# lyclyc52/SANeRF-HQ

Hardware: AMD Instinct MI355X
Metric: rays/s full render (800x800, hashgrid L=16 + 2x64 MLP) (higher is better)
Workload: dtype f32 arithmetic / f16 tables

## Files before the change

### include/sanerf_hip.h

```cpp
#ifndef SANERF_HIP_H
#define SANERF_HIP_H

#include <stddef.h>
#include <stdint.h>

#ifdef __cplusplus
extern "C" {
#endif

#define SN_MAX_LEVELS 32
#define SN_MAX_LAYERS 8
#define SN_MAX_STAGES 4
#define SN_ABI_VERSION 12

typedef void *sn_stream_t;

typedef enum {
    SN_OK = 0,
    SN_ERR_INVALID = -1,
    SN_ERR_UNSUPPORTED = -2,
    SN_ERR_HIP = -3,
    SN_ERR_WORKSPACE = -4,
    SN_ERR_WINDOW = -5
} sn_status;
// ... 249 lines not shown
    float       *f_feat;
    uint32_t     head_stride;
    void        *workspace;
    size_t       workspace_bytes;
} sn_render_io;

size_t sn_rm_render_workspace_bytes(const sn_render_cfg *cfg, uint32_t N, uint32_t tile_w);
int sn_rm_render_rays(const sn_render_cfg *cfg, const sn_render_io *io, sn_stream_t stream);
typedef struct sn_launch_info {
    char     final_kernel[64];
    uint32_t workgroups, lds_bytes, dense_levels, gathers_per_wave_sample, launches;
} sn_launch_info;
int sn_rm_last_launch_info(sn_launch_info *info);
int sn_rm_render_route_info(const sn_render_cfg *cfg, const sn_render_io *io, sn_launch_info *out);

int sn_rm_grid_composite(const float *xyzs, const float *weights, uint32_t N, uint32_t T, float bound,
                         const sn_grid_desc *grid, uint32_t tile_w, float *out, sn_stream_t stream);

size_t sn_mlp_wide_workspace_bytes(const sn_mlp_desc *mlp);
int sn_mlp_wide_overflow(int32_t *flag);
int sn_mlp_wide_forward(const sn_mlp_desc *mlp, const float *ln_weight, const float *ln_bias, float ln_eps,
                        const float *x, uint32_t N, float *out, void *workspace, size_t workspace_bytes,
                        sn_stream_t stream);

size_t sn_rm_mask_head_workspace_bytes(const sn_mlp_desc *mlp);
int sn_rm_mask_head(const float *xyzs, const float *extra, const float *weights, uint32_t N, uint32_t T, uint32_t E,
                    float bound, const sn_grid_desc *grid, const sn_mlp_desc *mlp, float *out,
                    void *workspace, size_t workspace_bytes, sn_stream_t stream);

int sn_mlp_wide_forward_train(const sn_mlp_desc *mlp, const float *x, uint32_t N, float *const *hidden, float *out, sn_stream_t stream);
// ... 58 lines not shown
```

### sanerf-hq_amd/_lib.py

```python
from __future__ import annotations

import ctypes as C
import os
import subprocess
from typing import Optional

import torch

_PKG = os.path.dirname(os.path.abspath(__file__))
LIB_PATH = os.environ.get("SN_LIB") or os.path.join(_PKG, "libsanerf_hip.so")
CSRC = os.path.join(_PKG, "csrc")

MAX_LEVELS, MAX_LAYERS, MAX_STAGES = 32, 8, 4
SN_F32, SN_F16 = 0, 1
LAYOUT_LBC, LAYOUT_BLC = 0, 1


class GridDesc(C.Structure):
    _fields_ = [("embeddings", C.c_void_p), ("table_dtype", C.c_int32), ("offsets", C.c_int32 * (MAX_LEVELS + 1)),
                ("D", C.c_uint32), ("C", C.c_uint32), ("L", C.c_uint32), ("S", C.c_float), ("H", C.c_uint32),
                ("gridtype", C.c_uint32), ("align_corners", C.c_uint32), ("interp", C.c_uint32)]


class MlpDesc(C.Structure):
# ... 29 lines not shown
                ("pred", C.c_uint64 * MASK_MAX_CLASSES), ("truth", C.c_uint64 * MASK_MAX_CLASSES)]


class SsimRecord(C.Structure):
    _fields_ = [("ssim_sum", C.c_double), ("last", C.c_double), ("images", C.c_uint64)]


class RenderTuning(C.Structure):
    _fields_ = [("mlp_mode", C.c_int32), ("per_sample_form", C.c_int32), ("densify", C.c_int32), ("linear_tile_order", C.c_int32),
                ("prop_sp_max_rays", C.c_int32), ("final_sp_max_rays", C.c_int32), ("feat_levels", C.c_int32), ("band_streams", C.c_int32), ("exact_early_out", C.c_int32), ("wave_tile", C.c_int32), ("prop_sp_lanes", C.c_int32), ("feat_patch", C.c_int32), ("prop_pair", C.c_int32), ("experiment", C.c_int32)]


class LaunchInfo(C.Structure):
    _fields_ = [("final_kernel", C.c_char * 64), ("workgroups", C.c_uint32), ("lds_bytes", C.c_uint32), ("dense_levels", C.c_uint32),
                ("gathers_per_wave_sample", C.c_uint32), ("launches", C.c_uint32)]


class RenderCfg(C.Structure):
    _fields_ = [("num_stages", C.c_uint32), ("num_steps", C.c_uint32 * MAX_STAGES),
                ("prop_grid", GridDesc * MAX_STAGES), ("prop_mlp", MlpDesc * MAX_STAGES),
                ("grid", GridDesc), ("grid_mlp", MlpDesc), ("view_mlp", MlpDesc),
                ("sh_degree", C.c_uint32), ("aabb", C.c_float * 6), ("min_near", C.c_float), ("bound", C.c_float),
                ("contract", C.c_int32), ("last_sample_opaque", C.c_int32), ("bg_color", C.c_float),
                ("feat_grid", GridDesc), ("with_feat", C.c_int32), ("early_stop_eps", C.c_float), ("mlp_exact_fp32", C.c_int32),
                ("compact_live", C.c_int32), ("tuning", RenderTuning)]


class RenderIO(C.Structure):
    _fields_ = [("rays_o", C.c_void_p), ("rays_d", C.c_void_p), ("cam_near_far", C.c_void_p),
                ("N", C.c_uint32), ("tile_w", C.c_uint32),
# ... 74 lines not shown
    "sn_rm_mask_nll": (_int, [_vp, _vp, _u32, _u32, _f32, _vp, _vp, _vp]),
    "sn_rm_ray_pair_select": (_int, [_vp, _vp, _u32, _u32, _u32, _vp, _vp]),
    "sn_rm_ray_pair_rgb_loss": (_int, [_vp, _vp, _int, _vp, _u32, _u32, _u32, _u32, _f32, _f32, _f32, _int, _f32, _vp, _vp, _vp, _vp, _vp]),
    "sn_rm_mask_error": (_int, [_vp, _int, _vp, _u32, _u32, _f32, _f32, _vp, _vp]),
    "sn_rm_error_map_update": (_int, [_vp, _int, _vp, _vp, _u32, _vp, _u32, _u32, _f32, _f32, _u32, _u32, _vp, _vp, _vp, _vp]),
    "sn_rm_mask_output": (_int, [_vp, _u32, _u32, _vp, _u32, _vp, _u32, _int, _int, _f32, _vp, _vp, _vp, _vp, _vp, _vp, _vp]),
    "sn_rm_mask_eval_accumulate": (_int, [_vp, _vp, _u32, _u32, _u32, _f32, _vp, _vp, _vp]),
    "sn_rm_image_sqerr_accumulate": (_int, [_vp, _u32, _vp, _u32, _u32, _vp, _vp, _vp]),
    "sn_rm_image_ssim_accumulate": (_int, [_vp, _u32, _vp, _u32, _u32, _u32, _f32, _vp, _vp, _vp]),
    "sn_rm_feature_distill_workspace_bytes": (C.c_size_t, [_u32, _u32, _u32, _u32, _u32]),
    "sn_rm_feature_distill_loss": (_int, [_vp, _u32, _u32, _u32, _u32, _vp, _u32, _u32, _f32, _vp, _vp, _vp, _vp, _vp, C.c_size_t, _vp]),
    "sn_rm_feature_map": (_int, [_vp, _u32, _u32, _u32, _u32, _u32, _u32, _vp, _vp]),
    "sn_rm_debug_occupancy": (_int, [_vp, _vp, _int]),
    "sn_rm_last_launch_info": (_int, [_vp]),
    "sn_rm_render_route_info": (_int, [C.POINTER(RenderCfg), C.POINTER(RenderIO), _vp]),
    "sn_debug_eval": (_int, [_int, _vp, _vp, _u32, _vp, _vp]),
}

EXPORTED_SYMBOLS = tuple(_SIGNATURES)

_lib = None


def build(force: bool = False) -> str:
    srcs = [os.path.join(CSRC, f) for f in os.listdir(CSRC) if f.endswith((".hip", ".h", ".inc"))]
    srcs.append(os.path.join(os.path.dirname(_PKG), "include", "sanerf_hip.h"))
    stale = force or not os.path.exists(LIB_PATH) or os.path.getmtime(LIB_PATH) < max(os.path.getmtime(s) for s in srcs)
    if stale:
        subprocess.check_call(["make", "-C", CSRC, "-j4"] + (["-B"] if force else []))
    return LIB_PATH
# ... 54 lines not shown
```

### sanerf-hq_amd/csrc/render.hip

```cpp
#include "sn_common.h"
#include "sh_basis.inc"

#include <float.h>
#include <stdlib.h>
#include <string.h>
#include <cstdio>
#include <map>
#include <mutex>
#include <type_traits>
#include <vector>

namespace sn {

typedef float floatx16 __attribute__((ext_vector_type(16)));

struct RayCommon {
    const float *rays_o, *rays_d, *cnf;
    uint32_t N;
    uint32_t W;
    uint32_t rows;
    uint32_t Npad;
    float aabb[6];
    float min_near, bound;
    int contract, last_opaque;
// ... 2958 lines not shown
struct WorkspacePlan {
    BandPlan bands;
    size_t pair_main = 0, pair_prop[SN_MAX_STAGES] = {};
    size_t pair_floats = 0, slot_floats = 0;
    size_t head_floats() const { return (size_t)PACK_FLOATS + pair_floats; }
    size_t bytes() const { return ((size_t)bands.slots * slot_floats + head_floats()) * sizeof(float); }
};
struct RenderRoute {
    GridLevels gl_prop[SN_MAX_STAGES], gl_main, gl_feat;
    bool is_main = false, is_any = false;
    AnyShape any;
    int mlp_mode = MLP_F16X3, mlp_np = 3;
    bool use_cmp = false;
    int Kmain = -1;
    int Kv_main = 0;
    float stop_cum = 0.0f;
    WorkspacePlan ws;
    FinalRoute fin;
    FeatRoute feat;
    uint32_t chunks = 0;
    ChunkRoute full, last;
};

static WorkspacePlan plan_workspace(const sn_render_cfg *cfg, uint32_t N, uint32_t W) {
    WorkspacePlan w;
    w.bands = band_plan(cfg, N, W);
    const uint32_t nc = w.bands.chunk < N ? w.bands.chunk : N;
    w.slot_floats = stage_scratch_floats(cfg, blocks_for(nc, W, tile_log2w(cfg)) * 256u);
    w.pair_floats = w.pair_main = pair_floats_of(&cfg->grid, (uint64_t)N * cfg->num_steps[cfg->num_stages - 1], cfg->tuning.densify);
    for (uint32_t k = 0; k + 1 < cfg->num_stages; ++k) w.pair_floats += w.pair_prop[k] = pair_floats_of(&cfg->prop_grid[k]);
// ... 2 lines not shown

static int check_io_pointers(const sn_render_cfg *cfg, const sn_render_io *io) {
    SN_REQUIRE(io->rays_o && io->rays_d, "render_rays: rays must be device pointers");
    if (io->skip_final) SN_REQUIRE(cfg->num_stages >= 2 && (cfg->num_stages > SN_MAX_STAGES  || io->bins[cfg->num_stages - 1]) && !cfg->with_feat,
                                   "render_rays: skip_final needs >= 2 stages, io->bins[last] for the resampled bins, and no feature stage");
    else SN_REQUIRE(io->image && io->depth && io->weights_sum, "render_rays: outputs must be device pointers");
    return SN_OK;
}

static void plan_final(const sn_render_cfg *cfg, const sn_render_io *io, RenderRoute *r) {
    const uint32_t S = cfg->num_stages;
    const bool f16 = cfg->grid.table_dtype == SN_F16;
    const int dp = dense_prefix(r->gl_main);
    const uint64_t main_samples = (uint64_t)io->N * cfg->num_steps[S - 1];
    r->Kv_main = r->is_any ? 0 : dp;
    const bool have_pairs = !r->is_any && dp > 0 && r->ws.pair_main != 0;
    r->Kmain = have_pairs && final_lv_fits(r->gl_main, dp, 2u * (f16 ? 2u : 4u)) ? dp : -1;
    if (cfg->compact_live && r->mlp_mode == MLP_F16X3 && !cfg->with_feat && !io->xyzs_last && !io->geo_feat_last && !io->skip_final &&
        io->bins0_ray_stride == 0) {
        bool any_dbg = false;
        for (uint32_t k = 1; k < S; ++k) any_dbg = any_dbg || io->u_ray_stride[k] != 0;
        for (uint32_t k = 0; k < S; ++k) any_dbg = any_dbg || io->bins[k] || io->weights[k] || io->sigmas[k] || io->inds[k];
        r->use_cmp = !any_dbg && dp == 5 && r->Kmain == 5;
    }
    if (io->skip_final) return;
    const bool dbg_last = io->bins[S - 1] || io->weights[S - 1] || io->sigmas[S - 1] || io->xyzs_last || io->geo_feat_last;
    const bool per_sample_out = dbg_last || cfg->with_feat;
    r->stop_cum = (cfg->early_stop_eps > 0.0f && cfg->early_stop_eps < 1.0f && !per_sample_out) ? -logf(cfg->early_stop_eps) : 0.0f;
    auto lv_gathers = [&](int kd) -> uint32_t { return (uint32_t)kd * (f16 ? 2u : 4u) + (uint32_t)(16 - kd) * 8u; };
    FinalRoute &f = r->fin;
    f.f16 = f16;
    f.aux = cfg->with_feat || r->stop_cum > 0.0f;
    f.eo = cfg->tuning.exact_early_out == 2;
    const int xp = experiment_of(cfg);
    const bool f16x3 = r->mlp_mode == MLP_F16X3;
    if (r->is_any) {
        f.family = FinalRoute::ANY; f.name = "k_final_stage_any";
        f.lds = (size_t)(2u * r->any.rows + (r->any.dg[r->any.ng] - 1u)) * 256u * sizeof(float);
        f.dense = 0; f.gathers = cfg->grid.L * 8u;
    } else if (r->use_cmp) {
        f.family = FinalRoute::CMP; f.name = "k_final_stage_cmp"; f.K = 5; f.lds = LDS_F16X3; f.dense = 5; f.gathers = lv_gathers(5);
    } else if (f16x3 && r->Kmain == 5 && !f.aux && !per_sample_out && xp == SN_EXP_ROLE_SPLIT) {
        f.family = FinalRoute::RS; f.name = "k_final_stage_rs"; f.K = 5; f.dense = 5; f.gathers = lv_gathers(5);
    } else if (f16x3 && r->Kmain == 5 && !dbg_last && lt_enabled(cfg)) {
        const bool l0 = f16 && (uint64_t)r->gl_main.res[0] * r->gl_main.res[0] * r->gl_main.res[0] <= (uint64_t)L0_MAX_ROWS && xp == SN_EXP_LDS_LEVEL0;
        if (!f.aux && !cfg->compact_live) r->Kv_main = densify_levels(r->gl_main, 5, main_samples, f16, cfg->tuning.densify);
        const bool dens = r->Kv_main == 7 && !l0 && final_lv_fits(r->gl_main, 7, 2u * (f16 ? 2u : 4u));
        f.family = l0 ? FinalRoute::LT_L0 : FinalRoute::LT;
        f.K = dens ? 7 : 5;
        f.name = l0 ? "k_final_stage<lt,K=5,lds-level0>" : dens ? "k_final_stage<lt,K=7>" : f.aux ? "k_final_stage<lt,K=5,aux>" : "k_final_stage<lt,K=5>";
        f.dense = f.K; f.gathers = lv_gathers(f.K) - (l0 ? 2u : 0u);
        if (f16 && !f.eo && r->mlp_np == 1 && !f.aux && !l0) f.np = 1;
        f.lds = l0 ? LDS_F16X3_L0 : (xp == SN_EXP_FINAL_ONE_WG && !dens && f.np == 3) ? (size_t)(84 * 1024) : LDS_F16X3;
    } else if (f16x3) {
        f.family = FinalRoute::PER_SAMPLE; f.K = r->Kmain == 5 ? 5 : -1; f.lds = LDS_F16X3;
        f.name = r->Kmain == 5 ? "k_final_stage<per-sample,K=5>" : "k_final_stage<per-sample,generic>";
        f.dense = r->Kmain; f.gathers = r->Kmain == 5 ? lv_gathers(5) : (uint32_t)dp * 4u + (16u - (uint32_t)dp) * 8u;
    } else if (r->mlp_mode == MLP_F32) {
        f.family = FinalRoute::MFMA32; f.name = "k_final_stage<mfma32>"; f.aux = true; f.lds = LDS_MFMA32; f.dense = -1; f.gathers = 16u * 8u;
    } else {
        f.family = FinalRoute::VALU; f.name = "k_final_stage<valu>"; f.aux = true; f.lds = LDS_VALU; f.dense = -1; f.gathers = 16u * 8u;
// ... 38 lines not shown
        sp.lds = final_sp_lds_floats(1u << spl_log2) * sizeof(float);
        sp.dense = r.Kmain; sp.gathers = r.Kmain == 5 ? (uint32_t)5 * (f.f16 ? 2u : 4u) + 11u * 8u : 16u * 8u;
        f = sp;
    }
    return c;
}

static void plan_chunks(const sn_render_cfg *cfg, const sn_render_io *io, RenderRoute *r) {
    const uint32_t chunk = r->ws.bands.chunk;
    r->chunks = div_up(io->N, chunk);
    r->full = plan_chunk(cfg, io, *r, io->N < chunk ? io->N : chunk);
    const uint32_t n_last = io->N - (r->chunks - 1u) * chunk;
    r->last = n_last == r->full.n ? r->full : plan_chunk(cfg, io, *r, n_last);
}

static int plan_render(const sn_render_cfg *cfg, const sn_render_io *io, RenderRoute *r) {
    SN_REQUIRE(io->out_stride == 0u || io->out_stride >= 5u, "render_rays: out_stride %u must be 0 (dense outputs) or at least 5 floats (rgb | depth | weights_sum per row)", io->out_stride);
    SN_REQUIRE(io->head_stride == 0u || (io->f_image && io->head_stride >= 31u + 4u && !io->skip_final),
               "render_rays: head_stride %u needs f_image and room for f_image | rgb | depth (>= 35 floats per row)", io->head_stride);
    SN_REQUIRE(cfg->tuning.wave_tile >= 0 && cfg->tuning.wave_tile <= 5, "render_rays: tuning.wave_tile %d outside 0..5", cfg->tuning.wave_tile);
    SN_REQUIRE(!(experiment_of(cfg) == SN_EXP_ROLE_SPLIT && cfg->tuning.wave_tile != 0 && cfg->tuning.wave_tile != 3), "render_rays: the role-split experiment is built for 8x8 wave tiles (tuning.wave_tile 0 or 3)");
    const uint32_t S = cfg->num_stages;
    SN_REQUIRE(S >= 1 && S <= SN_MAX_STAGES, "render_rays: num_stages=%u outside 1..%d", S, SN_MAX_STAGES);
    for (uint32_t k = 0; k < S; ++k) SN_REQUIRE(cfg->num_steps[k] >= 1, "render_rays: num_steps[%u] must be >= 1", k);
    SN_REQUIRE(cfg->sh_degree == 4, "render_rays: fused path is built for SH degree 4 (network.py:97), got %u", cfg->sh_degree);
    if (io->tile_w) SN_REQUIRE(io->N % io->tile_w == 0, "render_rays: N=%u is not a multiple of tile_w=%u", io->N, io->tile_w);
    SN_REQUIRE(io->bins0_ray_stride == 0 || (io->bins0_table && io->bins0_ray_stride >= cfg->num_steps[0] + 1u),
               "render_rays: bins0_ray_stride=%u needs bins0_table and at least num_steps[0]+1=%u values per ray", io->bins0_ray_stride, cfg->num_steps[0] + 1u);
    for (uint32_t k = 1; k < S; ++k)
        SN_REQUIRE(io->u_ray_stride[k] == 0 || (io->u_table[k] && io->u_ray_stride[k] >= cfg->num_steps[k] + 1u),
                   "render_rays: u_ray_stride[%u]=%u needs u_table[%u] and at least num_steps[%u]+1=%u values per ray", k, io->u_ray_stride[k], k, k, cfg->num_steps[k] + 1u);
// ... 174 lines not shown
        if (lg == 4u) return k_feat_stage<TT, C, 4, true>;
        if (lg == 2u) return k_feat_stage<TT, C, 2, true>;
        return k_feat_stage<TT, C, 1, true>;
    }
    if (lg == 4u) return k_feat_stage<TT, C, 4>;
    if (lg == 2u) return k_feat_stage<TT, C, 2>;
    return k_feat_stage<TT, C, 1>;
}
static FeatKern feat_kernel(const FeatRoute &ft, bool patch) {
    switch (ft.C) {
        case 8: return ft.f16 ? feat_kernel_of<__half, 8>(ft.lg, patch) : feat_kernel_of<float, 8>(ft.lg, patch);
        case 4: return ft.f16 ? feat_kernel_of<__half, 4>(ft.lg, patch) : feat_kernel_of<float, 4>(ft.lg, patch);
        default: return ft.f16 ? feat_kernel_of<__half, 2>(ft.lg, patch) : feat_kernel_of<float, 2>(ft.lg, patch);
    }
}
}

extern "C" {

size_t sn_rm_render_workspace_bytes(const sn_render_cfg *cfg, uint32_t N, uint32_t tile_w) {
    if (!cfg || N == 0 || cfg->num_stages < 1 || cfg->num_stages > SN_MAX_STAGES) return (size_t)PACK_FLOATS * sizeof(float);
    return plan_workspace(cfg, N, tile_w).bytes();
}

int sn_rm_render_route_info(const sn_render_cfg *cfg, const sn_render_io *io, sn_launch_info *out) {
    SN_REQUIRE(cfg && io && out, "render_route_info: cfg/io/out is NULL");
    *out = sn_launch_info{};
    if (io->N == 0) return SN_OK;
    int rc = check_io_pointers(cfg, io);
    if (rc) return rc;
    RenderRoute route;
    rc = plan_render(cfg, io, &route);
    if (rc) return rc;
    if (io->skip_final) return SN_OK;
    note_final(route.last.fin, out);
    out->launches = route.chunks;
    return SN_OK;
}

int sn_rm_render_rays(const sn_render_cfg *cfg, const sn_render_io *io, sn_stream_t stream) {
    SN_REQUIRE(cfg && io, "render_rays: cfg/io is NULL");
    if (io->N == 0) return SN_OK;
    g_launch = sn_launch_info{};
    int rc = check_io_pointers(cfg, io);
    if (rc) return rc;
    RenderRoute route;
    rc = plan_render(cfg, io, &route);
    if (rc) return rc;
    SN_REQUIRE(io->workspace != nullptr, "render_rays: workspace is NULL");
    SN_REQUIRE(table_aligned(io->workspace), "render_rays: workspace must be 16-byte aligned");
    if (io->workspace_bytes / sizeof(float) < route.ws.bytes() / sizeof(float)) {
        set_error("render_rays: workspace too small (%zu bytes, need %zu)", io->workspace_bytes, route.ws.bytes());
        return SN_ERR_WORKSPACE;
    }
    const uint32_t S = cfg->num_stages, W = io->tile_w;
    const hipStream_t st_main = (hipStream_t)stream;
    const GridLevels &gl_main = route.gl_main;
    float *pack = reinterpret_cast<float *>(io->workspace);
    float *pair_mem = pack + PACK_FLOATS;
    float *scratch = pair_mem + route.ws.pair_floats;

    if (route.mlp_mode != MLP_VALU && !route.is_any) {
        ProfScope ps(st_main, PK_PACK);
        if (route.mlp_mode == MLP_F16X3)
            rc = launch(k_pack_grid_mlp_f16, dim3(PACK16_VECS * 64 / 256), dim3(256), 0, st_main, cfg->grid_mlp.weight[0], cfg->grid_mlp.weight[1],
                        cfg->grid_mlp.weight[2], reinterpret_cast<uint4 *>(pack));
        else
            rc = launch(k_pack_grid_mlp, dim3(PACK_FLOATS / 256), dim3(256), 0, st_main, cfg->grid_mlp.weight[0], cfg->grid_mlp.weight[1], cfg->grid_mlp.weight[2], pack);
        if (rc) return rc;
        SN_LAUNCH_CHECK("k_pack_grid_mlp");
    }
    PairTab pairs, prop_pairs[SN_MAX_STAGES];
    {
        float *cursor = pair_mem;
        auto pack_pairs = [&](const sn_grid_desc *d, const GridLevels &gl, PairTab &pt, int Kp, size_t fl) -> int {
            pt.base = nullptr;
            for (int l = 0; l < 8; ++l) pt.off[l] = 0;
            if (fl == 0 || Kp <= 0) return SN_OK;
            pair_layout(gl, Kp, pt.off);
            pt.base = cursor;
            cursor += fl;
            uint32_t max_rows = 0;
            for (int l = 0; l < Kp; ++l) { const uint32_t r3 = gl.res[l] * gl.res[l] * gl.res[l]; if (r3 > max_rows) max_rows = r3; }
            const dim3 gp(div_up(max_rows, 256), (uint32_t)Kp);
            const int rcl = d->table_dtype == SN_F16 ? launch(k_pack_pairs<__half>, gp, dim3(256), 0, st_main, (const __half *)d->embeddings, gl, pt, (uint32_t)Kp)
                                                     : launch(k_pack_pairs<float>, gp, dim3(256), 0, st_main, (const float *)d->embeddings, gl, pt, (uint32_t)Kp);
            if (rcl) return rcl;
            SN_LAUNCH_CHECK("k_pack_pairs");
            return SN_OK;
        };
        ProfScope ps(st_main, PK_PACK);
        rc = pack_pairs(&cfg->grid, gl_main, pairs, route.Kv_main, route.ws.pair_main);
        if (rc) return rc;
        for (uint32_t k = 0; k + 1 < S; ++k) {
            rc = pack_pairs(&cfg->prop_grid[k], route.gl_prop[k], prop_pairs[k], dense_prefix(route.gl_prop[k]), route.ws.pair_prop[k]);
            if (rc) return rc;
        }
    }

    BandFork fork(st_main, route.ws.bands.slots == 2u);
    if (route.ws.bands.slots == 2u && !fork.side) {
        route.ws.bands.slots = 1u;
        plan_chunks(cfg, io, &route);
    }
    const uint32_t chunk = route.ws.bands.chunk;
    for (uint32_t ci = 0; ci < route.chunks; ++ci) {
        const uint32_t first = ci * chunk;
        const ChunkRoute &cr = ci + 1u < route.chunks ? route.full : route.last;
        const uint32_t n = cr.n, Npad = cr.Npad;
        const uint32_t slot = fork.side ? (ci & 1u) : 0u;
        const hipStream_t st = slot ? fork.side : st_main;
        RayCommon rays;
// ... 90 lines not shown
                ft.level0 = 0;
                rc = launch(feat_kernel(feat, true), dim3(cr.nblk, feat.patch_levels / feat.lg), dim3(256), 0, st, ft);
                if (rc) return rc;
            }
            if (feat.patch_levels < gf.L) {
                ft.level0 = feat.patch_levels;
                rc = launch(feat_kernel(feat, false), dim3(cr.nblk, (gf.L - feat.patch_levels) / feat.lg), dim3(256), 0, st, ft);
                if (rc) return rc;
            }
            SN_LAUNCH_CHECK("k_feat_stage");
        }
    }
    return SN_OK;
}

}
```

### sanerf-hq_amd/raymarching/raymarching.py

```python
from __future__ import annotations

import ctypes as C
import os
import warnings
from typing import Dict, List, Optional, Sequence

import numpy as np
import torch
from torch.autograd import Function

from .. import _lib


class Tuning:
    FIELDS = ("mlp_mode", "per_sample_form", "densify", "linear_tile_order", "prop_sp_max_rays", "final_sp_max_rays", "feat_levels", "band_streams", "exact_early_out", "wave_tile", "prop_sp_lanes", "feat_patch", "prop_pair", "experiment")

    def __init__(self, **kw):
        for f in self.FIELDS:
            setattr(self, f, 0)
        for k, v in kw.items():
            if k not in self.FIELDS:
                raise TypeError(f"Tuning: unknown field {k!r} (fields: {', '.join(self.FIELDS)})")
            setattr(self, k, int(v))

# ... 890 lines not shown
        if feat_encoder is not None:
            _fill_grid(cfg.feat_grid, feat_encoder, table_of(feat_encoder))
            cfg.with_feat = 1
            self.feat_dim = feat_encoder.output_dim
        cfg.early_stop_eps = float(early_stop_eps)
        cfg.compact_live = int(bool(compact_live))
        self.cfg = cfg
        self._range_model = model
        self._range_versions = None
        self.activation_bound = 0.0
        self.check_range()
        self.num_steps = [int(t) for t in num_steps]
        self.geo = int(getattr(model, "geom_feat_dim", list(model.grid_mlp.net)[-1].weight.shape[0] - 1))
        self.ncol = self.geo + model.view_encoder.output_dim
        self._ws: Optional[torch.Tensor] = None

    @torch.no_grad()
    def check_range(self) -> None:
        m = self._range_model
        tensors = [m.grid.embeddings] + [lin.weight for lin in m.grid_mlp.net]
        versions = tuple((t.data_ptr(), t._version) for t in tensors)
        if versions == self._range_versions:
            return
        self._range_versions = versions
        layers = list(m.grid_mlp.net)
        stats = [m.grid.embeddings.detach().abs().max().float()]
        stats += [lin.weight.detach().float().abs().sum(dim=1).max() for lin in layers[:-1]]
        stats += [lin.weight.detach().abs().max().float() for lin in layers]
        vals = torch.stack(stats).tolist()
        bound = worst = vals[0]
        for row_l1 in vals[1:len(layers)]:
            bound = row_l1 * bound
            worst = max(worst, bound)
        wmax = max(vals[len(layers):]) if layers else 0.0
        if any(v != v for v in vals):
            worst = float("nan")
        self.activation_bound = max(worst, wmax)
        exact = not (self.activation_bound < FP16_SPLIT_LIMIT)
        if exact and not self.cfg.mlp_exact_fp32:
            warnings.warn(f"fused render: activations of the 32-64-64-16 MLP are only bounded by {self.activation_bound:.3g} "
                          f"(>= {FP16_SPLIT_LIMIT:.0f}): using the exact fp32 matrix-core path instead of split-fp16")
        self.cfg.mlp_exact_fp32 = int(exact)

    def invalidate_range(self) -> None:
        self._range_versions = None

    @torch.no_grad()
    def refresh_tables(self) -> None:
        for src, copy in self.copies:
            copy.copy_(src.detach())

    def workspace(self, N: int, tile_w: int, device) -> torch.Tensor:
        (self.tuning or tuning).write(self.cfg.tuning)
        need = int(_lib.lib().sn_rm_render_workspace_bytes(C.byref(self.cfg), N, tile_w))
        if self._ws is None or self._ws.numel() < need or self._ws.device != torch.device(device):
            self._ws = torch.empty(need, dtype=torch.uint8, device=device)
        return self._ws


def _fill_io(plan: RenderPlan, io, N: int, tile_w: int, want, u_tables, bins0_table, skip_final: bool, packed, head_input: bool, tuning, buf, table):
    io.N, io.tile_w = N, int(tile_w)
    if bins0_table is not None:
        b0, io.bins0_table = table(bins0_table)
        if b0.dim() == 2:
            if b0.shape != (N, plan.num_steps[0] + 1):
# ... 41 lines not shown
    if head_input and plan.cfg.with_feat and not skip_final:
        io.f_feat = buf("head_input", (N, plan.feat_dim + plan.ncol + 4))
        io.f_image, io.head_stride = io.f_feat + 4 * plan.feat_dim, plan.feat_dim + plan.ncol + 4
    else:
        if "f_image" in want:
            io.f_image = buf("f_image", (N, plan.ncol))
        if plan.cfg.with_feat and not skip_final:
            io.f_feat = buf("f_feat", (N, plan.feat_dim))
    eff = tuning or plan.tuning or globals()["tuning"]
    eff.write(plan.cfg.tuning)
    return eff


def route_info(plan: RenderPlan, N: int, tile_w: int = 0, want: Sequence[str] = (), u_tables: Optional[Dict[int, torch.Tensor]] = None,
               bins0_table: Optional[torch.Tensor] = None, skip_final: bool = False, tuning: Optional["Tuning"] = None,
               packed: Optional[torch.Tensor] = None, head_input: bool = False) -> dict:
    io = _lib.RenderIO()
    stand_in = 64
    io.rays_o = io.rays_d = stand_in
    _fill_io(plan, io, int(N), tile_w, want, u_tables, bins0_table, skip_final, packed, head_input, tuning,
             lambda name, shape, dtype=torch.float32: stand_in, lambda t: (t, stand_in))
    info = _lib.LaunchInfo()
    _lib.check(_lib.lib().sn_rm_render_route_info(C.byref(plan.cfg), C.byref(io), C.byref(info)), "route_info")
    return dict(final_kernel=info.final_kernel.decode(), workgroups=int(info.workgroups), lds_bytes=int(info.lds_bytes),
                dense_levels=int(info.dense_levels), gathers_per_wave_sample=int(info.gathers_per_wave_sample), launches=int(info.launches))


def render_rays(plan: RenderPlan, rays_o, rays_d, cam_near_far=None, bg_color: float = 1.0, tile_w: int = 0,
                want: Sequence[str] = (), u_tables: Optional[Dict[int, torch.Tensor]] = None,
                bins0_table: Optional[torch.Tensor] = None, out: Optional[Dict[str, torch.Tensor]] = None,
                skip_final: bool = False, tuning: Optional["Tuning"] = None, packed: Optional[torch.Tensor] = None,
                head_input: bool = False):
    rays_o, rays_d = _flat3(rays_o), _flat3(rays_d)
    N = rays_o.shape[0]
    device = rays_o.device
    io = _lib.RenderIO()
    res: Dict[str, torch.Tensor] = {} if out is None else out
    keep: List[torch.Tensor] = []

    def buf(name, shape, dtype=torch.float32):
        t = res.get(name)
        if t is None or tuple(t.shape) != tuple(shape) or t.dtype != dtype or t.device != device or not t.is_contiguous():
            t = torch.empty(shape, device=device, dtype=dtype)
            res[name] = t
        return _lib.dev(t, name, dtype)

    def table(t):
# ... 14 lines not shown
                and packed.is_contiguous() and packed.device == device):
            raise RuntimeError(f"render_rays: packed must be a contiguous fp32 [{N}, >=5] tensor on {device}, got {tuple(packed.shape)} {packed.dtype}")
        res["image"], res["depth"], res["weights_sum"] = packed[:, :3], packed[:, 3], packed[:, 4]
    eff = _fill_io(plan, io, N, tile_w, want, u_tables, bins0_table, skip_final, packed, head_input, tuning, buf, table)
    S = plan.cfg.num_stages
    if io.head_stride:
        hb = res["head_input"]
        res["f_feat"], res["f_image"] = hb[:, :plan.feat_dim], hb[:, plan.feat_dim:plan.feat_dim + plan.ncol]
    need = int(_lib.lib().sn_rm_render_workspace_bytes(C.byref(plan.cfg), N, int(tile_w)))
    ws = plan.workspace(N, int(tile_w), device)
    if ws.numel() < need:
        plan._ws = ws = torch.empty(need, dtype=torch.uint8, device=device)
    eff.write(plan.cfg.tuning)
    io.workspace, io.workspace_bytes = ws.data_ptr(), ws.numel()
    plan.cfg.bg_color = float(bg_color)
    _lib.check(_lib.lib().sn_rm_render_rays(C.byref(plan.cfg), C.byref(io), _lib.stream()), "render_rays")
    if "weights_last" in set(want) and not skip_final:
        res["weights_last"] = res[f"weights{S - 1}"]
    return res
```

Before: 102.0 million.

## Cache packed MLP weights and pair tables across render calls

Adds a prepared-state API that packs the grid MLP weights and dense-level pair tables once into a persistent buffer, keyed by a hash of the grid and weight configuration. Render calls reuse this buffer instead of launching the pack kernels every time. The Python plan invalidates the cache when tensor versions change or tables are refreshed. The risks are stale state if the invalidation misses an in-place update, and a change in densify level choice, because the prepared path decides it without the real sample count.

```diff
diff --git a/include/sanerf_hip.h b/include/sanerf_hip.h
--- a/include/sanerf_hip.h
+++ b/include/sanerf_hip.h
@@ -287,6 +287,21 @@
 int sn_rm_last_launch_info(sn_launch_info *info);
 int sn_rm_render_route_info(const sn_render_cfg *cfg, const sn_render_io *io, sn_launch_info *out);
 
+typedef struct sn_render_prepared {
+    void    *base;
+    size_t   bytes;
+    uint64_t key;
+    int32_t  main_K;
+    int32_t  reserved;
+    size_t   pair_base[SN_MAX_STAGES + 1];
+    size_t   pair_floats[SN_MAX_STAGES + 1];
+    uint32_t pair_off[SN_MAX_STAGES + 1][8];
+} sn_render_prepared;
+size_t sn_rm_render_prepared_bytes(const sn_render_cfg *cfg);
+int sn_rm_render_prepare(const sn_render_cfg *cfg, void *prepared, size_t prepared_bytes, sn_render_prepared *out, sn_stream_t stream);
+int sn_rm_render_rays_prepared(const sn_render_cfg *cfg, const sn_render_io *io, const sn_render_prepared *prep, sn_stream_t stream);
+int sn_rm_render_route_info_prepared(const sn_render_cfg *cfg, const sn_render_io *io, const sn_render_prepared *prep, sn_launch_info *out);
+
 int sn_rm_grid_composite(const float *xyzs, const float *weights, uint32_t N, uint32_t T, float bound,
                          const sn_grid_desc *grid, uint32_t tile_w, float *out, sn_stream_t stream);
 
diff --git a/sanerf-hq_amd/_lib.py b/sanerf-hq_amd/_lib.py
--- a/sanerf-hq_amd/_lib.py
+++ b/sanerf-hq_amd/_lib.py
@@ -67,6 +67,12 @@
 class LaunchInfo(C.Structure):
     _fields_ = [("final_kernel", C.c_char * 64), ("workgroups", C.c_uint32), ("lds_bytes", C.c_uint32), ("dense_levels", C.c_uint32),
                 ("gathers_per_wave_sample", C.c_uint32), ("launches", C.c_uint32)]
+
+
+class RenderPrepared(C.Structure):
+    _fields_ = [("base", C.c_void_p), ("bytes", C.c_size_t), ("key", C.c_uint64), ("main_K", C.c_int32), ("reserved", C.c_int32),
+                ("pair_base", C.c_size_t * (MAX_STAGES + 1)), ("pair_floats", C.c_size_t * (MAX_STAGES + 1)),
+                ("pair_off", (C.c_uint32 * 8) * (MAX_STAGES + 1))]
 
 
 class RenderCfg(C.Structure):
@@ -171,6 +177,10 @@
     "sn_rm_debug_occupancy": (_int, [_vp, _vp, _int]),
     "sn_rm_last_launch_info": (_int, [_vp]),
     "sn_rm_render_route_info": (_int, [C.POINTER(RenderCfg), C.POINTER(RenderIO), _vp]),
+    "sn_rm_render_prepared_bytes": (C.c_size_t, [C.POINTER(RenderCfg)]),
+    "sn_rm_render_prepare": (_int, [C.POINTER(RenderCfg), _vp, C.c_size_t, C.POINTER(RenderPrepared), _vp]),
+    "sn_rm_render_rays_prepared": (_int, [C.POINTER(RenderCfg), C.POINTER(RenderIO), C.POINTER(RenderPrepared), _vp]),
+    "sn_rm_render_route_info_prepared": (_int, [C.POINTER(RenderCfg), C.POINTER(RenderIO), C.POINTER(RenderPrepared), _vp]),
     "sn_debug_eval": (_int, [_int, _vp, _vp, _u32, _vp, _vp]),
 }
 
diff --git a/sanerf-hq_amd/csrc/render.hip b/sanerf-hq_amd/csrc/render.hip
--- a/sanerf-hq_amd/csrc/render.hip
+++ b/sanerf-hq_amd/csrc/render.hip
@@ -2996,6 +2996,7 @@
     bool use_cmp = false;
     int Kmain = -1;
     int Kv_main = 0;
+    int prepK = -1;
     float stop_cum = 0.0f;
     WorkspacePlan ws;
     FinalRoute fin;
@@ -3028,7 +3029,8 @@
     const int dp = dense_prefix(r->gl_main);
     const uint64_t main_samples = (uint64_t)io->N * cfg->num_steps[S - 1];
     r->Kv_main = r->is_any ? 0 : dp;
-    const bool have_pairs = !r->is_any && dp > 0 && r->ws.pair_main != 0;
+    const bool prepared = r->prepK >= 0;
+    const bool have_pairs = !r->is_any && dp > 0 && (prepared ? r->prepK >= dp : r->ws.pair_main != 0);
     r->Kmain = have_pairs && final_lv_fits(r->gl_main, dp, 2u * (f16 ? 2u : 4u)) ? dp : -1;
     if (cfg->compact_live && r->mlp_mode == MLP_F16X3 && !cfg->with_feat && !io->xyzs_last && !io->geo_feat_last && !io->skip_final &&
         io->bins0_ray_stride == 0) {
@@ -3058,7 +3060,7 @@
         f.family = FinalRoute::RS; f.name = "k_final_stage_rs"; f.K = 5; f.dense = 5; f.gathers = lv_gathers(5);
     } else if (f16x3 && r->Kmain == 5 && !dbg_last && lt_enabled(cfg)) {
         const bool l0 = f16 && (uint64_t)r->gl_main.res[0] * r->gl_main.res[0] * r->gl_main.res[0] <= (uint64_t)L0_MAX_ROWS && xp == SN_EXP_LDS_LEVEL0;
-        if (!f.aux && !cfg->compact_live) r->Kv_main = densify_levels(r->gl_main, 5, main_samples, f16, cfg->tuning.densify);
+        if (!f.aux && !cfg->compact_live) r->Kv_main = prepared ? r->prepK : densify_levels(r->gl_main, 5, main_samples, f16, cfg->tuning.densify);
         const bool dens = r->Kv_main == 7 && !l0 && final_lv_fits(r->gl_main, 7, 2u * (f16 ? 2u : 4u));
         f.family = l0 ? FinalRoute::LT_L0 : FinalRoute::LT;
         f.K = dens ? 7 : 5;
@@ -3127,7 +3129,8 @@
     r->last = n_last == r->full.n ? r->full : plan_chunk(cfg, io, *r, n_last);
 }
 
-static int plan_render(const sn_render_cfg *cfg, const sn_render_io *io, RenderRoute *r) {
+static int plan_render(const sn_render_cfg *cfg, const sn_render_io *io, RenderRoute *r, int prepK = -1) {
+    r->prepK = prepK;
     SN_REQUIRE(io->out_stride == 0u || io->out_stride >= 5u, "render_rays: out_stride %u must be 0 (dense outputs) or at least 5 floats (rgb | depth | weights_sum per row)", io->out_stride);
     SN_REQUIRE(io->head_stride == 0u || (io->f_image && io->head_stride >= 31u + 4u && !io->skip_final),
                "render_rays: head_stride %u needs f_image and room for f_image | rgb | depth (>= 35 floats per row)", io->head_stride);
@@ -3332,6 +3335,124 @@
         default: return ft.f16 ? feat_kernel_of<__half, 2>(ft.lg, patch) : feat_kernel_of<float, 2>(ft.lg, patch);
     }
 }
+
+static int launch_packs(const sn_render_cfg *cfg, const RenderRoute &route, int Kmain, float *pack, size_t main_floats, const size_t *prop_floats,
+                        hipStream_t st, PairTab &pairs, PairTab *prop_pairs) {
+    int rc = SN_OK;
+    if (route.mlp_mode != MLP_VALU && !route.is_any) {
+        ProfScope ps(st, PK_PACK);
+        if (route.mlp_mode == MLP_F16X3)
+            rc = launch(k_pack_grid_mlp_f16, dim3(PACK16_VECS * 64 / 256), dim3(256), 0, st, cfg->grid_mlp.weight[0], cfg->grid_mlp.weight[1],
+                        cfg->grid_mlp.weight[2], reinterpret_cast<uint4 *>(pack));
+        else
+            rc = launch(k_pack_grid_mlp, dim3(PACK_FLOATS / 256), dim3(256), 0, st, cfg->grid_mlp.weight[0], cfg->grid_mlp.weight[1], cfg->grid_mlp.weight[2], pack);
+        if (rc) return rc;
+        SN_LAUNCH_CHECK("k_pack_grid_mlp");
+    }
+    float *cursor = pack + PACK_FLOATS;
+    auto pack_pairs = [&](const sn_grid_desc *d, const GridLevels &gl, PairTab &pt, int Kp, size_t fl) -> int {
+        pt.base = nullptr;
+        for (int l = 0; l < 8; ++l) pt.off[l] = 0;
+        if (fl == 0 || Kp <= 0) return SN_OK;
+        pair_layout(gl, Kp, pt.off);
+        pt.base = cursor;
+        cursor += fl;
+        uint32_t max_rows = 0;
+        for (int l = 0; l < Kp; ++l) { const uint32_t r3 = gl.res[l] * gl.res[l] * gl.res[l]; if (r3 > max_rows) max_rows = r3; }
+        const dim3 gp(div_up(max_rows, 256), (uint32_t)Kp);
+        const int rcl = d->table_dtype == SN_F16 ? launch(k_pack_pairs<__half>, gp, dim3(256), 0, st, (const __half *)d->embeddings, gl, pt, (uint32_t)Kp)
+                                                 : launch(k_pack_pairs<float>, gp, dim3(256), 0, st, (const float *)d->embeddings, gl, pt, (uint32_t)Kp);
+        if (rcl) return rcl;
+        SN_LAUNCH_CHECK("k_pack_pairs");
+        return SN_OK;
+    };
+    ProfScope ps(st, PK_PACK);
+    rc = pack_pairs(&cfg->grid, route.gl_main, pairs, Kmain, main_floats);
+    if (rc) return rc;
+    for (uint32_t k = 0; k + 1 < cfg->num_stages; ++k) {
+        rc = pack_pairs(&cfg->prop_grid[k], route.gl_prop[k], prop_pairs[k], dense_prefix(route.gl_prop[k]), prop_floats[k]);
+        if (rc) return rc;
+    }
+    return SN_OK;
+}
+
+static uint64_t prepared_key(const sn_render_cfg *cfg) {
+    uint64_t h = 1469598103934665603ull;
+    auto mix = [&](const void *p, size_t n) { const unsigned char *b = static_cast<const unsigned char *>(p); for (size_t i = 0; i < n; ++i) { h ^= b[i]; h *= 1099511628211ull; } };
+    auto u32 = [&](uint32_t v) { mix(&v, sizeof(v)); };
+    auto ptr = [&](const void *v) { const uint64_t a = (uint64_t)(uintptr_t)v; mix(&a, sizeof(a)); };
+    auto grid = [&](const sn_grid_desc &d) {
+        ptr(d.embeddings); u32((uint32_t)d.table_dtype); u32(d.D); u32(d.C); u32(d.L); mix(&d.S, sizeof(d.S)); u32(d.H);
+        u32(d.gridtype); u32(d.align_corners); u32(d.interp);
+        for (uint32_t l = 0; l <= d.L && l <= (uint32_t)SN_MAX_LEVELS; ++l) u32((uint32_t)d.offsets[l]);
+    };
+    const uint32_t S = cfg->num_stages <= SN_MAX_STAGES ? cfg->num_stages : 0u;
+    u32(cfg->num_stages);
+    for (uint32_t k = 0; k + 1 < S; ++k) grid(cfg->prop_grid[k]);
+    grid(cfg->grid);
+    u32(cfg->grid_mlp.num_layers);
+    for (uint32_t l = 0; l < cfg->grid_mlp.num_layers && l < (uint32_t)SN_MAX_LAYERS; ++l) { ptr(cfg->grid_mlp.weight[l]); u32(cfg->grid_mlp.dims[l]); u32(cfg->grid_mlp.dims[l + 1]); }
+    u32((uint32_t)cfg->mlp_exact_fp32); u32((uint32_t)cfg->tuning.mlp_mode); u32((uint32_t)cfg->tuning.densify);
+    u32(cfg->compact_live ? 1u : 0u); u32(cfg->with_feat ? 1u : 0u);
+    return h;
+}
+
+static int plan_prepared(const sn_render_cfg *cfg, sn_render_prepared *rec, RenderRoute *route) {
+    *rec = sn_render_prepared{};
+    alignas(16) static const float stand_in[4] = {};
+    float *const sp = const_cast<float *>(stand_in);
+    sn_render_io io = {};
+    io.rays_o = io.rays_d = sp;
+    io.N = 1;
+    io.image = io.depth = io.weights_sum = sp;
+    if (cfg->with_feat) io.f_feat = sp;
+    int rc = plan_render(cfg, &io, route);
+    if (rc) return rc;
+    const uint32_t S = cfg->num_stages;
+    const bool f16 = cfg->grid.table_dtype == SN_F16;
+    const uint32_t rb = 2u * (f16 ? 2u : 4u);
+    int K = 0;
+    if (!route->is_any && pair_floats_of(&cfg->grid) != 0) {
+        K = dense_prefix(route->gl_main);
+        if (K == 5 && route->Kmain == 5 && route->mlp_mode == MLP_F16X3 && !cfg->compact_live && !cfg->with_feat &&
+            densify_levels(route->gl_main, 5, ~0ull, f16, cfg->tuning.densify) == 7 && final_lv_fits(route->gl_main, 7, rb))
+            K = 7;
+    }
+    rec->main_K = K > 0 ? K : 0;
+    size_t cursor = PACK_FLOATS;
+    auto place = [&](int slot, const GridLevels &gl, int Kp, bool packable) {
+        uint32_t off[8];
+        const size_t fl = packable && Kp > 0 ? (size_t)pair_layout(gl, Kp, off) * 4u : 0u;
+        rec->pair_base[slot] = fl ? cursor : 0u;
+        rec->pair_floats[slot] = fl;
+        for (int l = 0; l < 8; ++l) rec->pair_off[slot][l] = fl ? off[l] : 0u;
+        cursor += fl;
+    };
+    place(SN_MAX_STAGES, route->gl_main, rec->main_K, rec->main_K > 0);
+    for (uint32_t k = 0; k + 1 < S; ++k) place((int)k, route->gl_prop[k], dense_prefix(route->gl_prop[k]), pair_floats_of(&cfg->prop_grid[k]) != 0);
+    rec->bytes = cursor * sizeof(float);
+    rec->key = prepared_key(cfg);
+    return SN_OK;
+}
+
+static int check_prepared(const sn_render_cfg *cfg, const sn_render_prepared *prep) {
+    SN_REQUIRE(prep->base != nullptr && prep->bytes >= (size_t)PACK_FLOATS * sizeof(float), "render_rays_prepared: the record holds no prepared state (sn_rm_render_prepare fills it)");
+    if (prep->key != prepared_key(cfg)) {
+        set_error("render_rays_prepared: the prepared state was built from another configuration (grid descriptors, table or weight pointers, table dtype, "
+                  "MLP mode or tuning.densify differ): prepare again");
+        return SN_ERR_INVALID;
+    }
+    return SN_OK;
+}
+
+static void prepared_tabs(const sn_render_prepared *prep, uint32_t S, PairTab &pairs, PairTab *prop_pairs) {
+    auto tab = [&](int slot, PairTab &pt) {
+        pt.base = prep->pair_floats[slot] ? reinterpret_cast<const float *>(prep->base) + prep->pair_base[slot] : nullptr;
+        for (int l = 0; l < 8; ++l) pt.off[l] = prep->pair_off[slot][l];
+    };
+    tab(SN_MAX_STAGES, pairs);
+    for (uint32_t k = 0; k + 1 < S; ++k) tab((int)k, prop_pairs[k]);
+}
 }
 
 extern "C" {
@@ -3356,14 +3477,20 @@
     return SN_OK;
 }
 
-int sn_rm_render_rays(const sn_render_cfg *cfg, const sn_render_io *io, sn_stream_t stream) {
+}
+
+static int render_impl(const sn_render_cfg *cfg, const sn_render_io *io, const sn_render_prepared *prep, sn_stream_t stream) {
     SN_REQUIRE(cfg && io, "render_rays: cfg/io is NULL");
     if (io->N == 0) return SN_OK;
     g_launch = sn_launch_info{};
     int rc = check_io_pointers(cfg, io);
     if (rc) return rc;
+    if (prep) {
+        rc = check_prepared(cfg, prep);
+        if (rc) return rc;
+    }
     RenderRoute route;
-    rc = plan_render(cfg, io, &route);
+    rc = plan_render(cfg, io, &route, prep ? prep->main_K : -1);
     if (rc) return rc;
     SN_REQUIRE(io->workspace != nullptr, "render_rays: workspace is NULL");
     SN_REQUIRE(table_aligned(io->workspace), "render_rays: workspace must be 16-byte aligned");
@@ -3374,46 +3501,15 @@
     const uint32_t S = cfg->num_stages, W = io->tile_w;
     const hipStream_t st_main = (hipStream_t)stream;
     const GridLevels &gl_main = route.gl_main;
-    float *pack = reinterpret_cast<float *>(io->workspace);
-    float *pair_mem = pack + PACK_FLOATS;
-    float *scratch = pair_mem + route.ws.pair_floats;
-
-    if (route.mlp_mode != MLP_VALU && !route.is_any) {
-        ProfScope ps(st_main, PK_PACK);
-        if (route.mlp_mode == MLP_F16X3)
-            rc = launch(k_pack_grid_mlp_f16, dim3(PACK16_VECS * 64 / 256), dim3(256), 0, st_main, cfg->grid_mlp.weight[0], cfg->grid_mlp.weight[1],
-                        cfg->grid_mlp.weight[2], reinterpret_cast<uint4 *>(pack));
-        else
-            rc = launch(k_pack_grid_mlp, dim3(PACK_FLOATS / 256), dim3(256), 0, st_main, cfg->grid_mlp.weight[0], cfg->grid_mlp.weight[1], cfg->grid_mlp.weight[2], pack);
+    float *pack = reinterpret_cast<float *>(prep ? prep->base : io->workspace);
+    float *scratch = reinterpret_cast<float *>(io->workspace) + route.ws.head_floats();
+
+    PairTab pairs, prop_pairs[SN_MAX_STAGES];
+    if (prep) {
+        prepared_tabs(prep, S, pairs, prop_pairs);
+    } else {
+        rc = launch_packs(cfg, route, route.Kv_main, pack, route.ws.pair_main, route.ws.pair_prop, st_main, pairs, prop_pairs);
         if (rc) return rc;
-        SN_LAUNCH_CHECK("k_pack_grid_mlp");
-    }
-    PairTab pairs, prop_pairs[SN_MAX_STAGES];
-    {
-        float *cursor = pair_mem;
-        auto pack_pairs = [&](const sn_grid_desc *d, const GridLevels &gl, PairTab &pt, int Kp, size_t fl) -> int {
-            pt.base = nullptr;
-            for (int l = 0; l < 8; ++l) pt.off[l] = 0;
-            if (fl == 0 || Kp <= 0) return SN_OK;
-            pair_layout(gl, Kp, pt.off);
-            pt.base = cursor;
-            cursor += fl;
-            uint32_t max_rows = 0;
-            for (int l = 0; l < Kp; ++l) { const uint32_t r3 = gl.res[l] * gl.res[l] * gl.res[l]; if (r3 > max_rows) max_rows = r3; }
-            const dim3 gp(div_up(max_rows, 256), (uint32_t)Kp);
-            const int rcl = d->table_dtype == SN_F16 ? launch(k_pack_pairs<__half>, gp, dim3(256), 0, st_main, (const __half *)d->embeddings, gl, pt, (uint32_t)Kp)
-                                                     : launch(k_pack_pairs<float>, gp, dim3(256), 0, st_main, (const float *)d->embeddings, gl, pt, (uint32_t)Kp);
-            if (rcl) return rcl;
-            SN_LAUNCH_CHECK("k_pack_pairs");
-            return SN_OK;
-        };
-        ProfScope ps(st_main, PK_PACK);
-        rc = pack_pairs(&cfg->grid, gl_main, pairs, route.Kv_main, route.ws.pair_main);
-        if (rc) return rc;
-        for (uint32_t k = 0; k + 1 < S; ++k) {
-            rc = pack_pairs(&cfg->prop_grid[k], route.gl_prop[k], prop_pairs[k], dense_prefix(route.gl_prop[k]), route.ws.pair_prop[k]);
-            if (rc) return rc;
-        }
     }
 
     BandFork fork(st_main, route.ws.bands.slots == 2u);
@@ -3534,4 +3630,67 @@
     return SN_OK;
 }
 
-}
+extern "C" {
+
+int sn_rm_render_rays(const sn_render_cfg *cfg, const sn_render_io *io, sn_stream_t stream) { return render_impl(cfg, io, nullptr, stream); }
+
+int sn_rm_render_rays_prepared(const sn_render_cfg *cfg, const sn_render_io *io, const sn_render_prepared *prep, sn_stream_t stream) {
+    SN_REQUIRE(prep, "render_rays_prepared: prep is NULL");
+    return render_impl(cfg, io, prep, stream);
+}
+
+size_t sn_rm_render_prepared_bytes(const sn_render_cfg *cfg) {
+    sn_render_prepared rec;
+    RenderRoute route;
+    if (!cfg || plan_prepared(cfg, &rec, &route) != SN_OK) return 0;
+    return rec.bytes;
+}
+
+int sn_rm_render_prepare(const sn_render_cfg *cfg, void *prepared, size_t prepared_bytes, sn_render_prepared *out, sn_stream_t stream) {
+    SN_REQUIRE(cfg && out, "render_prepare: cfg/out is NULL");
+    *out = sn_render_prepared{};
+    sn_render_prepared rec;
+    RenderRoute route;
+    int rc = plan_prepared(cfg, &rec, &route);
+    if (rc) return rc;
+    *out = rec;
+    SN_REQUIRE(prepared != nullptr, "render_prepare: the prepared buffer is NULL");
+    SN_REQUIRE(table_aligned(prepared), "render_prepare: the prepared buffer must be 16-byte aligned");
+    if (prepared_bytes < rec.bytes) {
+        set_error("render_prepare: prepared buffer too small (%zu bytes, need %zu)", prepared_bytes, rec.bytes);
+        return SN_ERR_WORKSPACE;
+    }
+    rec.base = prepared;
+    PairTab pairs, prop_pairs[SN_MAX_STAGES];
+    rc = launch_packs(cfg, route, rec.main_K, reinterpret_cast<float *>(prepared), rec.pair_floats[SN_MAX_STAGES], rec.pair_floats, (hipStream_t)stream, pairs, prop_pairs);
+    if (rc) return rc;
+    *out = rec;
+    return SN_OK;
+}
+
+int sn_rm_render_route_info_prepared(const sn_render_cfg *cfg, const sn_render_io *io, const sn_render_prepared *prep, sn_launch_info *out) {
+    SN_REQUIRE(cfg && io && out, "render_route_info: cfg/io/out is NULL");
+    *out = sn_launch_info{};
+    if (io->N == 0) return SN_OK;
+    int rc = check_io_pointers(cfg, io);
+    if (rc) return rc;
+    sn_render_prepared rec;
+    if (prep) {
+        rc = check_prepared(cfg, prep);
+        if (rc) return rc;
+    } else {
+        RenderRoute probe;
+        rc = plan_prepared(cfg, &rec, &probe);
+        if (rc) return rc;
+        prep = &rec;
+    }
+    RenderRoute route;
+    rc = plan_render(cfg, io, &route, prep->main_K);
+    if (rc) return rc;
+    if (io->skip_final) return SN_OK;
+    note_final(route.last.fin, out);
+    out->launches = route.chunks;
+    return SN_OK;
+}
+
+}
diff --git a/sanerf-hq_amd/raymarching/raymarching.py b/sanerf-hq_amd/raymarching/raymarching.py
--- a/sanerf-hq_amd/raymarching/raymarching.py
+++ b/sanerf-hq_amd/raymarching/raymarching.py
@@ -928,12 +928,72 @@
         self.geo = int(getattr(model, "geom_feat_dim", list(model.grid_mlp.net)[-1].weight.shape[0] - 1))
         self.ncol = self.geo + model.view_encoder.output_dim
         self._ws: Optional[torch.Tensor] = None
+        self._prep: Optional[dict] = None
+        self._prep_content = None
+        self._prep_hold = False
+
+    def _live_versions(self) -> tuple:
+        m = self._range_model
+        tensors = [m.grid.embeddings] + [lin.weight for lin in m.grid_mlp.net]
+        tensors += [m.prop_encoders[k].embeddings for k in range(self.cfg.num_stages - 1)]
+        return tuple((t.data_ptr(), t._version) for t in tensors)
+
+    def _drop_prepared(self) -> None:
+        self._prep = None
+        self._prep_hold = True
+
+    def prepared(self, skip_final: bool = False, commit: bool = True):
+        L = _lib.lib()
+        if not hasattr(L, "sn_rm_render_rays_prepared"):
+            return False, None
+        content = self._live_versions()
+        if self._prep_content is not None and content != self._prep_content:
+            if not commit:
+                return False, None
+            self._prep, self._prep_hold = None, True
+        if commit:
+            self._prep_content = content
+        t = self.cfg.tuning
+        key = (int(self.cfg.mlp_exact_fp32), int(t.mlp_mode), int(t.densify))
+        dev = self._range_model.grid.embeddings.device
+        stream = torch.cuda.current_stream()
+        capturing = torch.cuda.is_current_stream_capturing()
+        p = self._prep
+        if p is not None and (p["key"] != key or p["device"] != dev):
+            p = None
+            if commit and not (skip_final or capturing):
+                self._prep = None
+        if self._prep_hold and p is None:
+            if commit and not (skip_final or capturing):
+                self._prep_hold = False
+            return False, None
+        if p is None:
+            if skip_final or capturing:
+                return False, None
+            if not commit:
+                return True, None
+            need = int(L.sn_rm_render_prepared_bytes(C.byref(self.cfg)))
+            if need == 0:
+                raise RuntimeError("render_prepare: " + L.sn_last_error().decode())
+            buf = torch.empty(need, dtype=torch.uint8, device=dev)
+            rec = _lib.RenderPrepared()
+            _lib.check(L.sn_rm_render_prepare(C.byref(self.cfg), buf.data_ptr(), buf.numel(), C.byref(rec), stream.cuda_stream), "render_prepare")
+            ev = torch.cuda.Event()
+            ev.record(stream)
+            p = self._prep = dict(rec=rec, buf=buf, event=ev, streams={stream.cuda_stream}, key=key, device=dev)
+        elif stream.cuda_stream not in p["streams"]:
+            if capturing:
+                return False, None
+            if commit:
+                stream.wait_event(p["event"])
+                p["buf"].record_stream(stream)
+                p["streams"].add(stream.cuda_stream)
+        return True, p["rec"]
 
     @torch.no_grad()
     def check_range(self) -> None:
         m = self._range_model
-        tensors = [m.grid.embeddings] + [lin.weight for lin in m.grid_mlp.net]
-        versions = tuple((t.data_ptr(), t._version) for t in tensors)
+        versions = self._live_versions()[:1 + len(m.grid_mlp.net)]
         if versions == self._range_versions:
             return
         self._range_versions = versions
@@ -958,11 +1018,14 @@
 
     def invalidate_range(self) -> None:
         self._range_versions = None
+        self._drop_prepared()
 
     @torch.no_grad()
     def refresh_tables(self) -> None:
         for src, copy in self.copies:
             copy.copy_(src.detach())
+        if self.copies:
+            self._drop_prepared()
 
     def workspace(self, N: int, tile_w: int, device) -> torch.Tensor:
         (self.tuning or tuning).write(self.cfg.tuning)
@@ -1034,14 +1097,18 @@
 
 def route_info(plan: RenderPlan, N: int, tile_w: int = 0, want: Sequence[str] = (), u_tables: Optional[Dict[int, torch.Tensor]] = None,
                bins0_table: Optional[torch.Tensor] = None, skip_final: bool = False, tuning: Optional["Tuning"] = None,
-               packed: Optional[torch.Tensor] = None, head_input: bool = False) -> dict:
+               packed: Optional[torch.Tensor] = None, head_input: bool = False, stateless: bool = False) -> dict:
     io = _lib.RenderIO()
     stand_in = 64
     io.rays_o = io.rays_d = stand_in
     _fill_io(plan, io, int(N), tile_w, want, u_tables, bins0_table, skip_final, packed, head_input, tuning,
              lambda name, shape, dtype=torch.float32: stand_in, lambda t: (t, stand_in))
     info = _lib.LaunchInfo()
-    _lib.check(_lib.lib().sn_rm_render_route_info(C.byref(plan.cfg), C.byref(io), C.byref(info)), "route_info")
+    use, rec = (False, None) if stateless else plan.prepared(skip_final, commit=False)
+    if use:
+        _lib.check(_lib.lib().sn_rm_render_route_info_prepared(C.byref(plan.cfg), C.byref(io), C.byref(rec) if rec is not None else None, C.byref(info)), "route_info")
+    else:
+        _lib.check(_lib.lib().sn_rm_render_route_info(C.byref(plan.cfg), C.byref(io), C.byref(info)), "route_info")
     return dict(final_kernel=info.final_kernel.decode(), workgroups=int(info.workgroups), lds_bytes=int(info.lds_bytes),
                 dense_levels=int(info.dense_levels), gathers_per_wave_sample=int(info.gathers_per_wave_sample), launches=int(info.launches))
 
@@ -1050,7 +1117,7 @@
                 want: Sequence[str] = (), u_tables: Optional[Dict[int, torch.Tensor]] = None,
                 bins0_table: Optional[torch.Tensor] = None, out: Optional[Dict[str, torch.Tensor]] = None,
                 skip_final: bool = False, tuning: Optional["Tuning"] = None, packed: Optional[torch.Tensor] = None,
-                head_input: bool = False):
+                head_input: bool = False, stateless: bool = False):
     rays_o, rays_d = _flat3(rays_o), _flat3(rays_d)
     N = rays_o.shape[0]
     device = rays_o.device
@@ -1095,7 +1162,11 @@
     eff.write(plan.cfg.tuning)
     io.workspace, io.workspace_bytes = ws.data_ptr(), ws.numel()
     plan.cfg.bg_color = float(bg_color)
-    _lib.check(_lib.lib().sn_rm_render_rays(C.byref(plan.cfg), C.byref(io), _lib.stream()), "render_rays")
+    use, rec = plan.prepared(skip_final) if N and not stateless else (False, None)
+    if use:
+        _lib.check(_lib.lib().sn_rm_render_rays_prepared(C.byref(plan.cfg), C.byref(io), C.byref(rec), _lib.stream()), "render_rays")
+    else:
+        _lib.check(_lib.lib().sn_rm_render_rays(C.byref(plan.cfg), C.byref(io), _lib.stream()), "render_rays")
     if "weights_last" in set(want) and not skip_final:
         res["weights_last"] = res[f"weights{S - 1}"]
     return res
```

Result: no change. 102.9 million, median of 6 (+1.0%).
